# liuyuan-pal/NeRO

Measured on AMD Instinct MI355X. Metric: training rays/sec (Stage-I shape, 128 samples/ray), higher is better.
Workload: dtype f32 (dense layers: fp32 operands carried as exact / block-scaled 16-bit plane pairs or triples on the bf16/fp16 matrix pipe with fp32 accumulation, fp32-grade error; modes {'fwd': 'f16x3', 'tan': 'f16x3', 'bwd': 'f16x3', 'dw': 'f16x3'}); 1 GPU; GlossySynthetic 'bell' Stage-I shape, 4096 rays x (64+64+32) samples per GPU, training-schedule step 25000; rays_per_gpu=4096, parallelism=dp1, optimizer=adam(fused), streams=3, f16_paired_mask=3, fg_table=reference asset (tests/golden/fg_lut_ref.npz)

## Files before the change

### nero_amd/csrc/mlp_f16_util.h

```cpp
#pragma once

#ifdef F16_PHASE_TIMING
__device__ unsigned long long g_phase[16];
#define PH_DECL long long ph_t = clock64(), ph_acc[8] = {0, 0, 0, 0, 0, 0, 0, 0}
#define PH(k) do { __builtin_amdgcn_sched_barrier(0); const long long t_ = clock64(); ph_acc[k] += t_ - ph_t; ph_t = t_; __builtin_amdgcn_sched_barrier(0); } while (0)
#define PH_PARAM , long long& ph_t, long long (&ph_acc)[8]
#define PH_ARG , ph_t, ph_acc
#define PH_END do { if (threadIdx.x == 0) for (int k_ = 0; k_ < 8; ++k_) atomicAdd(&g_phase[k_], (unsigned long long)ph_acc[k_]); } while (0)
#else
#define PH_PARAM
#define PH_ARG
#define PH_DECL
#define PH(k)
#define PH_END
#endif

typedef _Float16 f16x8 __attribute__((ext_vector_type(8)));
typedef _Float16 f16x2 __attribute__((ext_vector_type(2)));
typedef float f32x2 __attribute__((ext_vector_type(2)));
typedef float f32x16 __attribute__((ext_vector_type(16)));

constexpr float BETA = 100.0f;
constexpr int SA = 528;
constexpr int PLANE_A = 64 * SA;
// ... 245 lines not shown
}
#define NERO_FENCE() __builtin_amdgcn_sched_barrier(0)
#ifdef GEMM_SGB
#define NERO_KSTEP_SCHED() do { \
    __builtin_amdgcn_sched_group_barrier(0x008, 1, 0); __builtin_amdgcn_sched_group_barrier(0x100, 1, 0); \
    __builtin_amdgcn_sched_group_barrier(0x008, 1, 0); __builtin_amdgcn_sched_group_barrier(0x100, 1, 0); \
    __builtin_amdgcn_sched_group_barrier(0x008, 1, 0); __builtin_amdgcn_sched_group_barrier(0x100, 1, 0); \
    __builtin_amdgcn_sched_group_barrier(0x008, 1, 0); __builtin_amdgcn_sched_group_barrier(0x100, 1, 0); \
    __builtin_amdgcn_sched_group_barrier(0x008, 1, 0); __builtin_amdgcn_sched_group_barrier(0x020, 1, 0); \
    __builtin_amdgcn_sched_group_barrier(0x008, 1, 0); __builtin_amdgcn_sched_group_barrier(0x020, 1, 0); } while (0)
#define NERO_MID_FENCE()
#else
#define NERO_KSTEP_SCHED()
#define NERO_MID_FENCE() NERO_FENCE()
#endif

#ifndef F16_PW_N
#define F16_PW_N 3
#endif
__device__ __forceinline__ void prefetch_w(WF& wa, WF& wb, WF& wc, const uint4* wp, int n, int from = 0) {
    const int last = n - 1;
    if (from <= 0) load_w(wa, wp, 0);
    if (from <= 1) load_w(wb, wp, 1 < last ? 1 : last);
    if (from <= 2) load_w(wc, wp, 2 < last ? 2 : last);
}
__device__ __forceinline__ void gemm_f16x3_loop(f32x16 (&aH)[2], f32x16 (&aL)[2], const uint4* wp, const char* xp, int half_bytes,
                                           int plane_bytes, int n, bool pre, WF& wa, WF& wb, WF& wc) {
    if (n <= 0) return;
    WF wd;
    XF xa, xb;
    const int last = n - 1;
#define NERO_CL(c) ((c) < last ? (c) : last)
    prefetch_w(wa, wb, wc, wp, n, pre ? F16_PW_N : 0);
    load_x(xa, xp, half_bytes, plane_bytes, 0);
    NERO_FENCE();
    for (int c = 0; c < n; c += 4) {
        load_w(wd, wp, NERO_CL(c + 3)); load_x(xb, xp, half_bytes, plane_bytes, NERO_CL(c + 1)); NERO_MID_FENCE();
        ops_compute(aH, aL, wa, xa); NERO_KSTEP_SCHED(); NERO_FENCE();
        if (c + 1 < n) {
            load_w(wa, wp, NERO_CL(c + 4)); load_x(xa, xp, half_bytes, plane_bytes, NERO_CL(c + 2)); NERO_MID_FENCE();
            ops_compute(aH, aL, wb, xb); NERO_KSTEP_SCHED(); NERO_FENCE();
        }
        if (c + 2 < n) {
            load_w(wb, wp, NERO_CL(c + 5)); load_x(xb, xp, half_bytes, plane_bytes, NERO_CL(c + 3)); NERO_MID_FENCE();
            ops_compute(aH, aL, wc, xa); NERO_KSTEP_SCHED(); NERO_FENCE();
        }
        if (c + 3 < n) {
            load_w(wc, wp, NERO_CL(c + 6)); load_x(xa, xp, half_bytes, plane_bytes, NERO_CL(c + 4)); NERO_MID_FENCE();
            ops_compute(aH, aL, wd, xb); NERO_KSTEP_SCHED(); NERO_FENCE();
        }
    }
#undef NERO_CL
}
__device__ __forceinline__ void gemm_f16x3_loop(f32x16 (&aH)[2], f32x16 (&aL)[2], const uint4* wp, const char* xp, int half_bytes,
                                           int plane_bytes, int n) {
    WF wa, wb, wc;
    gemm_f16x3_loop(aH, aL, wp, xp, half_bytes, plane_bytes, n, false, wa, wb, wc);
}


__device__ __forceinline__ void gemm_f16x3_lean(f32x16 (&aH)[2], f32x16 (&aL)[2], const uint4* wp, const char* xp, int half_bytes,
                                                int plane_bytes, int n) {
    if (n <= 0) return;
    WF w0, w1, w2;
    XF xa, xb;
    const int last = n - 1;
#define NERO_CL(c) ((c) < last ? (c) : last)
    load_w(w0, wp, 0);
    load_w(w1, wp, NERO_CL(1));
    load_x(xa, xp, half_bytes, plane_bytes, 0);
    NERO_FENCE();
    for (int c = 0; c < n; c += 6) {
        load_w(w2, wp, NERO_CL(c + 2)); load_x(xb, xp, half_bytes, plane_bytes, NERO_CL(c + 1)); NERO_FENCE();
        ops_compute(aH, aL, w0, xa); NERO_FENCE();
        if (c + 1 < n) { load_w(w0, wp, NERO_CL(c + 3)); load_x(xa, xp, half_bytes, plane_bytes, NERO_CL(c + 2)); NERO_FENCE(); ops_compute(aH, aL, w1, xb); NERO_FENCE(); }
        if (c + 2 < n) { load_w(w1, wp, NERO_CL(c + 4)); load_x(xb, xp, half_bytes, plane_bytes, NERO_CL(c + 3)); NERO_FENCE(); ops_compute(aH, aL, w2, xa); NERO_FENCE(); }
        if (c + 3 < n) { load_w(w2, wp, NERO_CL(c + 5)); load_x(xa, xp, half_bytes, plane_bytes, NERO_CL(c + 4)); NERO_FENCE(); ops_compute(aH, aL, w0, xb); NERO_FENCE(); }
        if (c + 4 < n) { load_w(w0, wp, NERO_CL(c + 6)); load_x(xb, xp, half_bytes, plane_bytes, NERO_CL(c + 5)); NERO_FENCE(); ops_compute(aH, aL, w1, xa); NERO_FENCE(); }
        if (c + 5 < n) { load_w(w1, wp, NERO_CL(c + 7)); load_x(xa, xp, half_bytes, plane_bytes, NERO_CL(c + 6)); NERO_FENCE(); ops_compute(aH, aL, w2, xb); NERO_FENCE(); }
    }
#undef NERO_CL
}

template <int V> struct IC { static constexpr int value = V; };
template <int I, int N, class F> __device__ __forceinline__ void static_for(F&& f) {
    if constexpr (I < N) { f(IC<I>{}); static_for<I + 1, N>(f); }
}
#ifndef GEMM_XD
#define GEMM_XD 1
#endif
#ifndef GEMM_WD
#define GEMM_WD 3
#endif
template <int N, class F>
__device__ __forceinline__ void gemm_f16x3_fixed_hook(f32x16 (&aH)[2], f32x16 (&aL)[2], const uint4* wp, const char* xp, int half_bytes,
                                                      int plane_bytes, F&& hook) {
    constexpr int XD = GEMM_XD, XN = XD + 1, WD = GEMM_WD, WN = WD + 1;
    WF w[WN];
    XF x[XN];
    static_for<0, WD>([&](auto c) { if (c.value < N) load_w(w[c.value], wp, c.value); });
    static_for<0, XD>([&](auto c) { if (c.value < N) load_x(x[c.value], xp, half_bytes, plane_bytes, c.value); });
    NERO_FENCE();
    static_for<0, N>([&](auto cc) {
        constexpr int c = cc.value;
        if (c + WD < N) load_w(w[(c + WD) % WN], wp, c + WD);
        if (c + XD < N) load_x(x[(c + XD) % XN], xp, half_bytes, plane_bytes, c + XD);
        hook(cc);
        NERO_MID_FENCE();
        ops_compute(aH, aL, w[c % WN], x[c % XN]);
        if (c + WD < N && c + XD < N) NERO_KSTEP_SCHED();
        NERO_FENCE();
    });
}
template <int N>
__device__ __forceinline__ void gemm_f16x3_fixed(f32x16 (&aH)[2], f32x16 (&aL)[2], const uint4* wp, const char* xp, int half_bytes,
                                                 int plane_bytes) {
    gemm_f16x3_fixed_hook<N>(aH, aL, wp, xp, half_bytes, plane_bytes, [](auto) {});
}

__device__ __forceinline__ void gemm_f16x3(f32x16 (&aH)[2], f32x16 (&aL)[2], const uint4* wp, const char* xp, int half_bytes,
                                           int plane_bytes, int n) {
#ifdef GEMM_ASSUME16
    gemm_f16x3_fixed<16>(aH, aL, wp, xp, half_bytes, plane_bytes); return;
#endif
    gemm_f16x3_loop(aH, aL, wp, xp, half_bytes, plane_bytes, n);
}

__device__ __forceinline__ void zero2(f32x16 (&acc)[2]) {
#pragma unroll
    for (int r = 0; r < 2; ++r)
#pragma unroll
        for (int v = 0; v < 16; ++v) acc[r][v] = 0.f;
}

#ifdef NERO_SHFL_LDS
__device__ __forceinline__ float max_xor32(float m) { return fmaxf(m, __shfl_xor(m, 32)); }
__device__ __forceinline__ unsigned other_half(unsigned v, int h) { (void)h; return __shfl_xor(v, 32); }
__device__ __forceinline__ float max_8lanes(float m) { m = fmaxf(m, __shfl_xor(m, 1)); m = fmaxf(m, __shfl_xor(m, 2)); return fmaxf(m, __shfl_xor(m, 4)); }
__device__ __forceinline__ float max_4lanes(float m) { m = fmaxf(m, __shfl_xor(m, 1)); return fmaxf(m, __shfl_xor(m, 2)); }
__device__ __forceinline__ float sum_8lanes(float s) { s += __shfl_xor(s, 1); s += __shfl_xor(s, 2); return s + __shfl_xor(s, 4); }
#else
__device__ __forceinline__ float max_xor32(float m) {
    const auto r = __builtin_amdgcn_permlane32_swap(__float_as_uint(m), __float_as_uint(m), false, false);
    return fmaxf(__uint_as_float(r[0]), __uint_as_float(r[1]));
}
__device__ __forceinline__ unsigned other_half(unsigned v, int h) {
    const auto r = __builtin_amdgcn_permlane32_swap(v, v, false, false);
    return h ? r[0] : r[1];
}
template <int CTRL> __device__ __forceinline__ float dpp_f32(float v) {
    return __uint_as_float(__builtin_amdgcn_update_dpp(0u, __float_as_uint(v), CTRL, 0xf, 0xf, true));
}
__device__ __forceinline__ float max_4lanes(float m) { m = fmaxf(m, dpp_f32<0xB1>(m)); return fmaxf(m, dpp_f32<0x4E>(m)); }
__device__ __forceinline__ float max_8lanes(float m) { m = max_4lanes(m); return fmaxf(m, dpp_f32<0x141>(m)); }
__device__ __forceinline__ float sum_8lanes(float s) { s += dpp_f32<0xB1>(s); s += dpp_f32<0x4E>(s); return s + dpp_f32<0x141>(s); }
#endif

__device__ __forceinline__ void publish_rowmax(float* rmax, float m0, float m1, int wave, int i, int h) {
    m0 = max_xor32(m0);
    m1 = max_xor32(m1);
    if (h == 0) { rmax[i * 8 + wave] = m0; rmax[(32 + i) * 8 + wave] = m1; }
}
__device__ __forceinline__ float row_max8(const float* rmax, int row) {
    const float4 a = *reinterpret_cast<const float4*>(rmax + row * 8);
    const float4 b = *reinterpret_cast<const float4*>(rmax + row * 8 + 4);
    return fmaxf(fmaxf(fmaxf(a.x, a.y), fmaxf(a.z, a.w)), fmaxf(fmaxf(b.x, b.y), fmaxf(b.z, b.w)));
// ... 81 lines not shown
```

### nero_amd/csrc/mlp_f16p.hip

```cpp
#include <hip/hip_runtime.h>
#include <stdint.h>
#include "../../include/nero_hip.h"
#include "common.h"
#include "mlp_split.h"

namespace {

#include "mlp_f16_util.h"

#ifndef P_PA_EARLY_A
#define P_PA_EARLY_A true
#endif
#ifndef P_PA_EARLY_B
#define P_PA_EARLY_B true
#endif

struct LdsP { char* actp; float* rs_main; float* rs_aux; float* rmax; float* wsc; char* scr; };
__device__ __forceinline__ LdsP carve_p(char* smem) {
    LdsP l;
    l.actp = smem;
    l.rs_main = reinterpret_cast<float*>(smem + 2 * PLANE_A);
    l.rs_aux = l.rs_main + 64;
    l.rmax = l.rs_aux + 64;
    l.wsc = l.rmax + 64 * 8;
    l.scr = reinterpret_cast<char*>(l.wsc + 32);
    return l;
}
#ifndef NERO_F16_PW_DEFAULT
#define NERO_F16_PW_DEFAULT 4
#endif
#ifndef P_LDS_EXTRA
#define P_LDS_EXTRA 0
#endif
inline int p_lds_bytes() { return 2 * PLANE_A + LDS_SMALL_BYTES + 4 * SCRP_BYTES + P_LDS_EXTRA; }

struct Ctx { LdsP S; int wave, lane, i, h, row0, n_rows; float* scr; };

template <int NW>
__device__ __forceinline__ void load_planes_scaled_p(char* planes, float* rs, const float* __restrict__ src, int ld, int k, int row0,
                                                     int n_rows, int tid) {
    constexpr int NV = 64 / NW;
    const int r = tid / NW, q = tid % NW;
    const int k16 = (k + 15) & ~15, q4 = k16 >> 2;
    int gr = row0 + r;
    gr = gr < n_rows ? gr : n_rows - 1;
    const float* rowp = src + (size_t)gr * ld;
    float4 v[NV];
    float m = 0.f;
#pragma unroll
    for (int j = 0; j < NV; ++j) {
        const int c4 = 4 * (q + NW * j);
        v[j] = make_float4(0.f, 0.f, 0.f, 0.f);
        if (c4 < k) v[j] = *reinterpret_cast<const float4*>(rowp + c4);
        m = fmaxf(m, amax4(v[j]));
    }
    m = NW == 8 ? max_8lanes(m) : max_4lanes(m);
    const int e = scale_exp(m);
    const float inv = pow2i(-e);
#pragma unroll
    for (int j = 0; j < NV; ++j)
        if (q + NW * j < q4) store_planes4h(planes + r * SA + (q + NW * j) * 8, PLANE_A, scale4(v[j], inv));
    if (q == 0) rs[r] = pow2i(e);
}

template <int NW>
__device__ __forceinline__ void aux_row_scales_p(float* rs, const float* __restrict__ src, int ld, int k, int row0, int n_rows, int tid) {
    const int r = tid / NW, q = tid % NW;
    int gr = row0 + r;
    gr = gr < n_rows ? gr : n_rows - 1;
    const float* rowp = src + (size_t)gr * ld;
    float m = 0.f;
    for (int c4 = 4 * q; c4 < k; c4 += 4 * NW) m = fmaxf(m, amax4(*reinterpret_cast<const float4*>(rowp + c4)));
    m = NW == 8 ? max_8lanes(m) : max_4lanes(m);
    if (q == 0) rs[r] = pow2i(scale_exp(m));
}

struct RawX { float4 a0, a1, b0, b1; };
__device__ __forceinline__ void load_raw(RawX& o, const float* p0, const float* p1, int c, int h, int k) {
    const int c0 = 16 * c + 8 * h;
    const float4 z = make_float4(0.f, 0.f, 0.f, 0.f);
    o.a0 = c0 < k ? *reinterpret_cast<const float4*>(p0 + c0) : z;
    o.a1 = c0 + 4 < k ? *reinterpret_cast<const float4*>(p0 + c0 + 4) : z;
    o.b0 = c0 < k ? *reinterpret_cast<const float4*>(p1 + c0) : z;
    o.b1 = c0 + 4 < k ? *reinterpret_cast<const float4*>(p1 + c0 + 4) : z;
}
__device__ __forceinline__ void split8(uint4& hp, uint4& lp, float4 a, float4 b, float inv) {
    split2h(a.x * inv, a.y * inv, hp.x, lp.x);
    split2h(a.z * inv, a.w * inv, hp.y, lp.y);
    split2h(b.x * inv, b.y * inv, hp.z, lp.z);
    split2h(b.z * inv, b.w * inv, hp.w, lp.w);
}
__device__ __forceinline__ void raw_to_x(XF& x, const RawX& r, float inv0, float inv1) {
    split8(x.xh0, x.xl0, r.a0, r.a1, inv0);
    split8(x.xh1, x.xl1, r.b0, r.b1, inv1);
}
__device__ __forceinline__ void gemm_aux_global(f32x16 (&aH)[2], f32x16 (&aL)[2], const uint4* wp, const float* __restrict__ aux, int ld,
                                                int k, int n, const Ctx& c, float inv0, float inv1) {
    if (n <= 0) return;
    int g0 = c.row0 + c.i, g1 = c.row0 + 32 + c.i;
    g0 = g0 < c.n_rows ? g0 : c.n_rows - 1;
    g1 = g1 < c.n_rows ? g1 : c.n_rows - 1;
    const float* p0 = aux + (size_t)g0 * ld;
    const float* p1 = aux + (size_t)g1 * ld;
    WF wa, wb;
    RawX ra, rb;
    XF x;
    load_w(wa, wp, 0);
    load_raw(ra, p0, p1, 0, c.h, k);
    for (int s = 0; s < n; s += 2) {
        if (s + 1 < n) { load_w(wb, wp, s + 1); load_raw(rb, p0, p1, s + 1, c.h, k); }
        NERO_FENCE();
        raw_to_x(x, ra, inv0, inv1);
        ops_compute(aH, aL, wa, x);
        NERO_FENCE();
        if (s + 1 < n) {
            if (s + 2 < n) { load_w(wa, wp, s + 2); load_raw(ra, p0, p1, s + 2, c.h, k); }
            NERO_FENCE();
            raw_to_x(x, rb, inv0, inv1);
            ops_compute(aH, aL, wb, x);
            NERO_FENCE();
        }
    }
}

template <int NW>
__device__ __forceinline__ void gemm_tile(f32x16 (&aH)[2], f32x16 (&aL)[2], float (&U)[2], const Ctx& c, int t, const float* w_main,
                                          const float* w_aux, float wsc_main, float wsc_aux, int sm, int sx, const float* aux, int ld_aux,
                                          int k_aux_cols) {
    if (sx > 0) {
        const float wsc = wsc_aux;
        const float ra0 = c.S.rs_aux[c.i], ra1 = c.S.rs_aux[32 + c.i];
        gemm_aux_global(aH, aL, reinterpret_cast<const uint4*>(reinterpret_cast<const char*>(w_aux) + HDR_BYTES) + (size_t)t * sx * 128 + c.lane,
                        aux, ld_aux, k_aux_cols, sx, c, 1.f / ra0, 1.f / ra1);
        U[0] = wsc * ra0;
        U[1] = wsc * ra1;
    }
    if (sm > 0) {
        const float wsc = wsc_main;
        const float u0 = wsc * c.S.rs_main[c.i], u1 = wsc * c.S.rs_main[32 + c.i];
        if (sx > 0) {
            const float r0 = U[0] / u0, r1 = U[1] / u1;
#pragma unroll
            for (int v = 0; v < 16; ++v) {
                aH[0][v] *= r0; aH[1][v] *= r1;
#ifdef F16_TWO_ACC
                aL[0][v] *= r0; aL[1][v] *= r1;
#endif
            }
        }
        U[0] = u0;
        U[1] = u1;
        const uint4* wp = reinterpret_cast<const uint4*>(reinterpret_cast<const char*>(w_main) + HDR_BYTES) + (size_t)t * sm * 128 + c.lane;
        if (NW == 8) gemm_f16x3_lean(aH, aL, wp, c.S.actp + c.i * SA + 16 * c.h, 32 * SA, PLANE_A, sm);
        else gemm_f16x3(aH, aL, wp, c.S.actp + c.i * SA + 16 * c.h, 32 * SA, PLANE_A, sm);
    }
}

template <int NW>
__device__ __forceinline__ void eval_head_p(const char* planes, const float* rs, const float* __restrict__ w, const float* __restrict__ b,
                                            float* __restrict__ out, int n_head, int hk, int row0, int tid) {
    const int q = tid & 7;
#pragma unroll
    for (int pass = 0; pass < 8 / NW; ++pass) {
        const int r = (tid >> 3) + 32 * pass;
        float s[4] = {0.f, 0.f, 0.f, 0.f};
        for (int c4 = 4 * q; c4 < hk; c4 += 32) {
            const float4 x = load_planes4h(planes + r * SA + c4 * 2, PLANE_A);
#pragma unroll
            for (int j = 0; j < 4; ++j)
                if (j < n_head) {
                    const float4 ww = *reinterpret_cast<const float4*>(w + j * NERO_HID + c4);
                    s[j] = fmaf(x.x, ww.x, fmaf(x.y, ww.y, fmaf(x.z, ww.z, fmaf(x.w, ww.w, s[j]))));
                }
        }
#pragma unroll
        for (int j = 0; j < 4; ++j) s[j] = sum_8lanes(s[j]);
        if (q == 0) {
            const float sc = rs[r];
#pragma unroll
            for (int j = 0; j < 4; ++j)
                if (j < n_head) out[(size_t)(row0 + r) * 4 + j] = s[j] * sc + (b ? b[j] : 0.f);
        }
    }
}

template <int NW>
__device__ __forceinline__ void commit_planes_p(const Ctx& c, const float4 (&v0)[2][4], const float4 (&v1)[2][4], bool live0, bool live1) {
    __syncthreads();
    const int e0 = scale_exp(row_max8(c.S.rmax, c.i)), e1 = scale_exp(row_max8(c.S.rmax, 32 + c.i));
    const float inv0 = pow2i(-e0), inv1 = pow2i(-e1);
    if (live0) {
        char* dst = c.S.actp + c.i * SA + (32 * c.wave + 4 * c.h) * 2;
#pragma unroll
        for (int g = 0; g < 4; ++g) {
            store_planes4h(dst + 16 * g, PLANE_A, scale4(v0[0][g], inv0));
            store_planes4h(dst + 32 * SA + 16 * g, PLANE_A, scale4(v0[1][g], inv1));
        }
    }
    if (NW == 4 && live1) {
        char* dst = c.S.actp + c.i * SA + (32 * (c.wave + NW) + 4 * c.h) * 2;
#pragma unroll
        for (int g = 0; g < 4; ++g) {
            store_planes4h(dst + 16 * g, PLANE_A, scale4(v1[0][g], inv0));
            store_planes4h(dst + 32 * SA + 16 * g, PLANE_A, scale4(v1[1][g], inv1));
        }
    }
    if (c.wave == 0 && c.h == 0) { c.S.rs_main[c.i] = pow2i(e0); c.S.rs_main[32 + c.i] = pow2i(e1); }
    __syncthreads();
}

template <int NW>
__device__ __forceinline__ Ctx make_ctx(char* smem, int n_rows) {
    Ctx c;
    c.S = carve_p(smem);
    c.lane = threadIdx.x & 63;
    c.wave = __builtin_amdgcn_readfirstlane(threadIdx.x >> 6);
    c.i = c.lane & 31;
    c.h = c.lane >> 5;
    c.row0 = blockIdx.x * 64;
    c.n_rows = n_rows;
    c.scr = reinterpret_cast<float*>(c.S.scr + c.wave * (NW == 8 ? SCRP_BYTES / 2 : SCRP_BYTES));
    return c;
}

template <int ACT>
__device__ __forceinline__ void fwd_values(const f32x16 (&aH)[2], const f32x16 (&aL)[2], const float4 (&bq)[4], const float (&U)[2],
                                           float4 (&val)[2][4], float (&m)[2]) {
#pragma unroll
    for (int r = 0; r < 2; ++r) {
        m[r] = 0.f;
#pragma unroll
        for (int g = 0; g < 4; ++g) {
            float4 v;
            v.x = act_fwd<ACT>(fmaf(ACCV(aH, aL, r, 4 * g), U[r], bq[g].x));
            v.y = act_fwd<ACT>(fmaf(ACCV(aH, aL, r, 4 * g + 1), U[r], bq[g].y));
            v.z = act_fwd<ACT>(fmaf(ACCV(aH, aL, r, 4 * g + 2), U[r], bq[g].z));
            v.w = act_fwd<ACT>(fmaf(ACCV(aH, aL, r, 4 * g + 3), U[r], bq[g].w));
            val[r][g] = v;
            m[r] = fmaxf(m[r], amax4(v));
        }
    }
}

template <int NW>
__device__ __forceinline__ void fwd_tile(const nero_fwd_chain& ch, const nero_fwd_layer& L, int l, const Ctx& c, int t, float4 (&val)[2][4],
                                         float (&m)[2] PH_PARAM) {
    m[0] = m[1] = 0.f;
    if (t < L.n_tiles) {
        f32x16 aH[2], aL[2];
        zero2(aH);
        zero2(aL);
        float4 bq[4];
        auto load_bias = [&]() {
#pragma unroll
            for (int g = 0; g < 4; ++g)
                bq[g] = L.bias ? *reinterpret_cast<const float4*>(L.bias + 32 * t + 8 * g + 4 * c.h) : make_float4(0.f, 0.f, 0.f, 0.f);
        };
        if (NW == 4) load_bias();
        float U[2] = {1.f, 1.f};
        PH(1);
        gemm_tile<NW>(aH, aL, U, c, t, L.w_main, L.w_aux, c.S.wsc[2 * l], c.S.wsc[2 * l + 1], L.k_main >> 4, L.k_aux >> 4, ch.aux, ch.ld_aux, ch.k_aux);
        if (NW == 8) { NERO_FENCE(); load_bias(); }
        PH(2);
        if (L.act == NERO_ACT_RELU) fwd_values<NERO_ACT_RELU>(aH, aL, bq, U, val, m);
        else if (L.act == NERO_ACT_SOFTPLUS100) fwd_values<NERO_ACT_SOFTPLUS100>(aH, aL, bq, U, val, m);
        else fwd_values<NERO_ACT_NONE>(aH, aL, bq, U, val, m);
        PH(3);
        if (L.save) {
            float* sblock = L.save + (size_t)c.row0 * NERO_HID + 32 * t;
            acc_to_global_rows<64 / NW>(c.scr, val[0], sblock, c.lane);
            acc_to_global_rows<64 / NW>(c.scr, val[1], sblock + (size_t)32 * NERO_HID, c.lane);
        }
        if (L.relu_mask) {
#pragma unroll
            for (int r = 0; r < 2; ++r) {
                unsigned bits = 0u;
#pragma unroll
                for (int g = 0; g < 4; ++g) {
                    bits |= (val[r][g].x > 0.f ? 1u : 0u) << (4 * g);
                    bits |= (val[r][g].y > 0.f ? 1u : 0u) << (4 * g + 1);
                    bits |= (val[r][g].z > 0.f ? 1u : 0u) << (4 * g + 2);
                    bits |= (val[r][g].w > 0.f ? 1u : 0u) << (4 * g + 3);
                }
                const unsigned other = other_half(bits, c.h);
                if (c.h == 0) L.relu_mask[(size_t)(c.row0 + 32 * r + c.i) * 8 + t] = bits | (other << 16);
            }
        }
    }
    publish_rowmax(c.S.rmax, m[0], m[1], t, c.i, c.h);
    PH(4);
}

template <int NW>
__global__ __launch_bounds__(NW * 64, NW / 2) void fwd_p_kernel(nero_fwd_chain ch, int n_rows) {
    extern __shared__ __attribute__((aligned(16))) char smem[];
    const Ctx c = make_ctx<NW>(smem, n_rows);
    const int tid = threadIdx.x;
    PH_DECL;
#ifdef F16_PHASE_TIMING
    const long long ph_start = ph_t;
#endif
    WscRegs wr;
    wsc_request(wr, ch, [](const nero_fwd_layer& Lx, const float*& pm, const float*& pa) { pm = Lx.k_main > 0 && Lx.n_tiles > 0 ? Lx.w_main : nullptr; pa = Lx.k_aux > 0 && Lx.n_tiles > 0 ? Lx.w_aux : nullptr; });
    if (ch.init) load_planes_scaled_p<NW>(c.S.actp, c.S.rs_main, ch.init, ch.ld_init, ch.k_init, c.row0, n_rows, tid);
    if (ch.aux) aux_row_scales_p<NW>(c.S.rs_aux, ch.aux, ch.ld_aux, ch.k_aux, c.row0, n_rows, tid);
    wsc_commit(c.S.wsc, wr, tid);
    __syncthreads();
    PH(0);
    for (int l = 0; l < ch.n_layers; ++l) {
        const nero_fwd_layer L = load_layer(ch, l);
        if (L.n_head > 0) eval_head_p<NW>(c.S.actp, c.S.rs_main, L.head_w, L.head_b, L.head_out, L.n_head, L.head_k, c.row0, tid);
        if (L.n_tiles == 0) continue;
        float4 v0[2][4], v1[2][4];
        float m0[2], m1[2];
        fwd_tile<NW>(ch, L, l, c, c.wave, v0, m0 PH_ARG);
        if (NW == 4) fwd_tile<NW>(ch, L, l, c, c.wave + NW, v1, m1 PH_ARG);
        commit_planes_p<NW>(c, v0, v1, c.wave < L.n_tiles, c.wave + NW < L.n_tiles);
        PH(5);
    }
#ifdef F16_PHASE_TIMING
    ph_acc[7] = clock64() - ph_start;
    ph_acc[6] = 0;
#endif
    PH_END;
}

template <int NW>
__device__ __forceinline__ void tan_tile(const nero_tan_chain& ch, const nero_tan_layer& L, int l, const Ctx& c, int t, float4 (&val)[2][4],
                                         float (&m)[2]) {
    m[0] = m[1] = 0.f;
    if (t < L.n_tiles) {
        const size_t goff = (size_t)(c.row0 + c.i) * NERO_HID + 32 * t + 4 * c.h;
        const size_t boff = (size_t)c.row0 * NERO_HID + 32 * t;
        const bool want_inj = L.inj != nullptr;
        f32x16 aH[2], aL[2];
        zero2(aH);
        zero2(aL);
        float U[2] = {1.f, 1.f};
        gemm_tile<NW>(aH, aL, U, c, t, L.w_main, L.w_aux, c.S.wsc[2 * l], c.S.wsc[2 * l + 1], L.k_main >> 4, L.k_aux >> 4, ch.aux, ch.ld_aux, ch.k_aux);
        NERO_FENCE();
        float4 pa[2][4], pg[2][4];
#pragma unroll
        for (int r = 0; r < 2; ++r)
#pragma unroll
            for (int g = 0; g < 4; ++g) {
                pa[r][g] = *reinterpret_cast<const float4*>(L.a_saved + goff + (size_t)r * 32 * NERO_HID + 8 * g);
                pg[r][g] = make_float4(0.f, 0.f, 0.f, 0.f);
            }
        if (want_inj) {
#pragma unroll
            for (int r = 0; r < 2; ++r)
#pragma unroll
                for (int g = 0; g < 4; ++g) pg[r][g] = *reinterpret_cast<const float4*>(L.gbar + goff + (size_t)r * 32 * NERO_HID + 8 * g);
        }
        float* scr = c.scr;
#pragma unroll
        for (int r = 0; r < 2; ++r) {
            const bool live = (c.row0 + 32 * r + c.i) < c.n_rows;
            float4 ijq[4], adq[4];
#pragma unroll
            for (int g = 0; g < 4; ++g) {
                const float4 a = pa[r][g], gb = pg[r][g];
                float4 ad, ij;
                tan_elem(a.x, ACCV(aH, aL, r, 4 * g) * U[r], gb.x, live, ad.x, ij.x);
                tan_elem(a.y, ACCV(aH, aL, r, 4 * g + 1) * U[r], gb.y, live, ad.y, ij.y);
                tan_elem(a.z, ACCV(aH, aL, r, 4 * g + 2) * U[r], gb.z, live, ad.z, ij.z);
                tan_elem(a.w, ACCV(aH, aL, r, 4 * g + 3) * U[r], gb.w, live, ad.w, ij.w);
                val[r][g] = ad;
                m[r] = fmaxf(m[r], amax4(ad));
                adq[g] = live ? ad : make_float4(0.f, 0.f, 0.f, 0.f);
                ijq[g] = ij;
            }
            acc_to_global_rows<64 / NW>(scr, adq, L.adot + boff + (size_t)r * 32 * NERO_HID, c.lane);
            if (want_inj) acc_to_global_rows<64 / NW>(scr, ijq, L.inj + boff + (size_t)r * 32 * NERO_HID, c.lane);
        }
    }
    publish_rowmax(c.S.rmax, m[0], m[1], t, c.i, c.h);
}

template <int NW>
__global__ __launch_bounds__(NW * 64, NW / 2) void tan_p_kernel(nero_tan_chain ch, int n_rows) {
    extern __shared__ __attribute__((aligned(16))) char smem[];
    const Ctx c = make_ctx<NW>(smem, n_rows);
    const int tid = threadIdx.x;
    WscRegs wr;
    wsc_request(wr, ch, [](const nero_tan_layer& Lx, const float*& pm, const float*& pa) { pm = Lx.k_main > 0 ? Lx.w_main : nullptr; pa = Lx.k_aux > 0 ? Lx.w_aux : nullptr; });
    if (ch.init) load_planes_scaled_p<NW>(c.S.actp, c.S.rs_main, ch.init, ch.ld_init, ch.k_init, c.row0, n_rows, tid);
    if (ch.aux) aux_row_scales_p<NW>(c.S.rs_aux, ch.aux, ch.ld_aux, ch.k_aux, c.row0, n_rows, tid);
    wsc_commit(c.S.wsc, wr, tid);
    __syncthreads();
    for (int l = 0; l < ch.n_layers; ++l) {
        const nero_tan_layer L = load_layer(ch, l);
        float4 v0[2][4], v1[2][4];
        float m0[2], m1[2];
        tan_tile<NW>(ch, L, l, c, c.wave, v0, m0);
        if (NW == 4) tan_tile<NW>(ch, L, l, c, c.wave + NW, v1, m1);
        commit_planes_p<NW>(c, v0, v1, c.wave < L.n_tiles, c.wave + NW < L.n_tiles);
    }
}

__device__ __forceinline__ void combine_acc(float4 (&gq)[2][4], const f32x16 (&aH)[2], const f32x16 (&aL)[2], const float (&u)[2]) {
#pragma unroll
    for (int r = 0; r < 2; ++r)
#pragma unroll
        for (int g = 0; g < 4; ++g)
            gq[r][g] = make_float4(ACCV(aH, aL, r, 4 * g) * u[r], ACCV(aH, aL, r, 4 * g + 1) * u[r],
                                   ACCV(aH, aL, r, 4 * g + 2) * u[r], ACCV(aH, aL, r, 4 * g + 3) * u[r]);
}

template <bool PA_EARLY, int NW, bool MASKS>
__device__ __forceinline__ void bwd_tile(const nero_bwd_chain& ch, const nero_bwd_layer& L, int l, const Ctx& c, int t, bool first, float rs0, float rs1,
                                         float4 (&val)[2][4], float (&m)[2]) {
    m[0] = m[1] = 0.f;
    const bool live_t = t < L.k_main_tiles;
    const int fbase = 32 * t + 4 * c.h;
    const size_t goff = (size_t)(c.row0 + c.i) * NERO_HID + fbase;
    const size_t boff = (size_t)c.row0 * NERO_HID + 32 * t;
    const int steps = L.n_out >> 4;
    const bool has_inj = !MASKS && !first && L.inj != nullptr;
    const char* xp = c.S.actp + c.i * SA + 16 * c.h;
    float4 pa[2][4];
    auto load_pa = [&]() {
        if (first || !live_t) return;
        if (MASKS && L.act_prev != NERO_ACT_RELU) return;
        if (MASKS || (L.mask_prev && L.act_prev == NERO_ACT_RELU)) {
#pragma unroll
            for (int r = 0; r < 2; ++r) {
                const unsigned bits = L.mask_prev[(size_t)(c.row0 + 32 * r + c.i) * 8 + t] >> (16 * c.h);
#pragma unroll
                for (int g = 0; g < 4; ++g)
                    pa[r][g] = make_float4((bits >> (4 * g)) & 1u ? 1.f : 0.f, (bits >> (4 * g + 1)) & 1u ? 1.f : 0.f,
                                           (bits >> (4 * g + 2)) & 1u ? 1.f : 0.f, (bits >> (4 * g + 3)) & 1u ? 1.f : 0.f);
            }
        } else if (!MASKS) {
#pragma unroll
            for (int r = 0; r < 2; ++r)
#pragma unroll
                for (int g = 0; g < 4; ++g) pa[r][g] = *reinterpret_cast<const float4*>(L.a_prev + goff + (size_t)r * 32 * NERO_HID + 8 * g);
        }
    };
    float4 gq[2][4];
    if (L.n_out > 0) {
        f32x16 aH[2], aL[2];
        if (ch.d_aux && L.w_aux_t && t < L.k_aux_tiles) {
            zero2(aH);
            zero2(aL);
            const float wsc = c.S.wsc[2 * l + 1];
            if (NW == 8) gemm_f16x3_lean(aH, aL, reinterpret_cast<const uint4*>(reinterpret_cast<const char*>(L.w_aux_t) + HDR_BYTES) + (size_t)t * steps * 128 + c.lane, xp, 32 * SA, PLANE_A, steps);
            else gemm_f16x3(aH, aL, reinterpret_cast<const uint4*>(reinterpret_cast<const char*>(L.w_aux_t) + HDR_BYTES) + (size_t)t * steps * 128 + c.lane,
                       xp, 32 * SA, PLANE_A, steps);
            const float u[2] = {wsc * rs0, wsc * rs1};
            combine_acc(gq, aH, aL, u);
#pragma unroll
            for (int r = 0; r < 2; ++r)
#pragma unroll
                for (int g = 0; g < 4; ++g) {
                    const int f = fbase + 8 * g;
                    if (f < ch.ld_daux) *reinterpret_cast<float4*>(ch.d_aux + (size_t)(c.row0 + 32 * r + c.i) * ch.ld_daux + f) = gq[r][g];
                }
        }
        if (!live_t || (first && !ch.d_init)) { publish_rowmax(c.S.rmax, 0.f, 0.f, t, c.i, c.h); return; }
        if (PA_EARLY) {
            load_pa();
            NERO_FENCE();
        }
        zero2(aH);
        zero2(aL);
        const float wsc = c.S.wsc[2 * l];
        if (NW == 8) gemm_f16x3_lean(aH, aL, reinterpret_cast<const uint4*>(reinterpret_cast<const char*>(L.w_main_t) + HDR_BYTES) + (size_t)t * steps * 128 + c.lane, xp, 32 * SA, PLANE_A, steps);
        else gemm_f16x3(aH, aL, reinterpret_cast<const uint4*>(reinterpret_cast<const char*>(L.w_main_t) + HDR_BYTES) + (size_t)t * steps * 128 + c.lane,
                   xp, 32 * SA, PLANE_A, steps);
        const float u[2] = {wsc * rs0, wsc * rs1};
        combine_acc(gq, aH, aL, u);
        if (first) {
            if (ch.d_init) {
                const int ldi = ch.ld_dinit;
#pragma unroll
                for (int r = 0; r < 2; ++r)
#pragma unroll
                    for (int g = 0; g < 4; ++g) {
                        const int f = fbase + 8 * g;
                        if (f < ldi) {
                            float4 v = gq[r][g];
                            float4* dstp = reinterpret_cast<float4*>(ch.d_init + (size_t)(c.row0 + 32 * r + c.i) * ldi + f);
                            if (ch.accumulate_dinit) { const float4 o = *dstp; v.x += o.x; v.y += o.y; v.z += o.z; v.w += o.w; }
                            *dstp = v;
                        }
                    }
            }
            return;
        }
    } else {
        if (!live_t) { publish_rowmax(c.S.rmax, 0.f, 0.f, t, c.i, c.h); return; }
        if (PA_EARLY) load_pa();
#pragma unroll
        for (int g = 0; g < 4; ++g) {
            gq[0][g] = scale4(load_planes4h(c.S.actp + c.i * SA + (fbase + 8 * g) * 2, PLANE_A), rs0);
            gq[1][g] = scale4(load_planes4h(c.S.actp + (32 + c.i) * SA + (fbase + 8 * g) * 2, PLANE_A), rs1);
        }
    }
    if (!PA_EARLY) {
        NERO_FENCE();
        load_pa();
    }
    float4 ijp[2][4];
#pragma unroll
    for (int r = 0; r < 2; ++r)
#pragma unroll
        for (int g = 0; g < 4; ++g) ijp[r][g] = make_float4(0.f, 0.f, 0.f, 0.f);
    if (L.act_prev == NERO_ACT_RELU) bwd_values_h<NERO_ACT_RELU, false>(gq, pa, goff, has_inj, L, c.row0, c.i, fbase, c.n_rows, val, m, ijp);
    else if (!MASKS && L.act_prev == NERO_ACT_SOFTPLUS100) bwd_values_h<NERO_ACT_SOFTPLUS100, false>(gq, pa, goff, has_inj, L, c.row0, c.i, fbase, c.n_rows, val, m, ijp);
    else bwd_values_h<NERO_ACT_NONE, false>(gq, pa, goff, has_inj, L, c.row0, c.i, fbase, c.n_rows, val, m, ijp);
    if (L.delta_prev) {
        acc_to_global_rows<64 / NW>(c.scr, val[0], L.delta_prev + boff, c.lane);
        acc_to_global_rows<64 / NW>(c.scr, val[1], L.delta_prev + boff + (size_t)32 * NERO_HID, c.lane);
    }
    publish_rowmax(c.S.rmax, m[0], m[1], t, c.i, c.h);
}

template <int NW, bool MASKS>
__global__ __launch_bounds__(NW * 64, NW / 2) void bwd_p_kernel(nero_bwd_chain ch, int n_rows) {
    extern __shared__ __attribute__((aligned(16))) char smem[];
    const Ctx c = make_ctx<NW>(smem, n_rows);
    const int tid = threadIdx.x;
    WscRegs wr;
    wsc_request(wr, ch, [](const nero_bwd_layer& Lx, const float*& pm, const float*& pa) { pm = Lx.n_out > 0 ? Lx.w_main_t : nullptr; pa = Lx.n_out > 0 ? Lx.w_aux_t : nullptr; });
    if (ch.dy) load_planes_scaled_p<NW>(c.S.actp, c.S.rs_main, ch.dy, ch.ld_dy, ch.k_dy, c.row0, n_rows, tid);
    else {
        for (int idx = tid; idx < 2 * PLANE_A / 16; idx += NW * 64) reinterpret_cast<uint4*>(c.S.actp)[idx] = make_uint4(0u, 0u, 0u, 0u);
        if (tid < 64) c.S.rs_main[tid] = 1.f;
    }
    wsc_commit(c.S.wsc, wr, tid);
    __syncthreads();
    for (int l = ch.n_layers - 1; l >= 0; --l) {
        const nero_bwd_layer L = load_layer(ch, l);
        const bool first = (L.a_prev == nullptr);
        if (first && ch.d_init == nullptr && !(ch.d_aux && L.w_aux_t)) break;
        if (first && L.n_out == 0) break;
        const float rs0 = c.S.rs_main[c.i], rs1 = c.S.rs_main[32 + c.i];
        float4 v0[2][4], v1[2][4];
        float m0[2], m1[2];
        bwd_tile<P_PA_EARLY_A, NW, MASKS>(ch, L, l, c, c.wave, first, rs0, rs1, v0, m0);
        if (NW == 4) bwd_tile<P_PA_EARLY_B, NW, MASKS>(ch, L, l, c, c.wave + NW, first, rs0, rs1, v1, m1);
        if (first) break;
        commit_planes_p<NW>(c, v0, v1, c.wave < L.k_main_tiles, c.wave + NW < L.k_main_tiles);
    }
}

}

#include <stdio.h>
#include <stdlib.h>
#ifdef F16_PHASE_TIMING
extern "C" int nero_debug_phases_p(unsigned long long* out16, int reset) {
    hipDeviceSynchronize();
    if (out16) hipMemcpyFromSymbol(out16, HIP_SYMBOL(g_phase), sizeof(unsigned long long) * 16);
    if (reset) { unsigned long long z[16] = {0}; hipMemcpyToSymbol(HIP_SYMBOL(g_phase), z, sizeof(z)); }
    return 0;
}
#endif
static void report_occupancy(const void* f, const char* name) {
    if (!getenv("NERO_DEBUG_OCC")) return;
    for (int lds = 32768; lds <= 81920; lds += 2048 * 3) {
        int nb = -1;
        hipError_t e = hipOccupancyMaxActiveBlocksPerMultiprocessor(&nb, f, 256, lds);
        fprintf(stderr, "[nero] %s: dynamic LDS %d -> %d workgroups per CU (err %d)\n", name, lds, nb, (int)e);
    }
// ... 58 lines not shown
```

Measured before the change: 148,300 rays/s.

## Compute paired output tiles in one GEMM pass sharing activation loads

When a wave owns two output tiles (NW==4), the forward and tangent chains now run a dual GEMM that loads each activation fragment once and feeds it to two weight streams and two accumulator sets, instead of two separate GEMM passes. Epilogues are factored out so both tiles reuse them. The goal is to halve activation LDS/global reads and the loop overhead per tile pair. The cost is doubled accumulator and weight-fragment registers, which may lower occupancy or cause spills. A small asm trick also keeps the bwd store indices in VGPRs.

```diff
diff --git a/nero_amd/csrc/mlp_f16_util.h b/nero_amd/csrc/mlp_f16_util.h
--- a/nero_amd/csrc/mlp_f16_util.h
+++ b/nero_amd/csrc/mlp_f16_util.h
@@ -351,6 +351,39 @@
 #undef NERO_CL
 }
 
+struct WF2 { WF a, b; };
+__device__ __forceinline__ void load_w2(WF2& o, const uint4* wp0, const uint4* wp1, int c) {
+    load_w(o.a, wp0, c);
+    load_w(o.b, wp1, c);
+}
+__device__ __forceinline__ void ops_compute2(f32x16 (&aH0)[2], f32x16 (&aL0)[2], f32x16 (&aH1)[2], f32x16 (&aL1)[2], const WF2& w, const XF& x) {
+    ops_compute(aH0, aL0, w.a, x);
+    ops_compute(aH1, aL1, w.b, x);
+}
+__device__ __forceinline__ void gemm_f16x3_dual(f32x16 (&aH0)[2], f32x16 (&aL0)[2], f32x16 (&aH1)[2], f32x16 (&aL1)[2], const uint4* wp0,
+                                                const uint4* wp1, const char* xp, int half_bytes, int plane_bytes, int n) {
+    if (n <= 0) return;
+    WF2 w0, w1, w2;
+    XF xa, xb;
+    const int last = n - 1;
+#define NERO_CL(c) ((c) < last ? (c) : last)
+#define NERO_K2(W, X) NERO_MID_FENCE(); ops_compute2(aH0, aL0, aH1, aL1, W, X); NERO_FENCE()
+    load_w2(w0, wp0, wp1, 0);
+    load_w2(w1, wp0, wp1, NERO_CL(1));
+    load_x(xa, xp, half_bytes, plane_bytes, 0);
+    NERO_FENCE();
+    for (int c = 0; c < n; c += 6) {
+        load_w2(w2, wp0, wp1, NERO_CL(c + 2)); load_x(xb, xp, half_bytes, plane_bytes, NERO_CL(c + 1)); NERO_K2(w0, xa);
+        if (c + 1 < n) { load_w2(w0, wp0, wp1, NERO_CL(c + 3)); load_x(xa, xp, half_bytes, plane_bytes, NERO_CL(c + 2)); NERO_K2(w1, xb); }
+        if (c + 2 < n) { load_w2(w1, wp0, wp1, NERO_CL(c + 4)); load_x(xb, xp, half_bytes, plane_bytes, NERO_CL(c + 3)); NERO_K2(w2, xa); }
+        if (c + 3 < n) { load_w2(w2, wp0, wp1, NERO_CL(c + 5)); load_x(xa, xp, half_bytes, plane_bytes, NERO_CL(c + 4)); NERO_K2(w0, xb); }
+        if (c + 4 < n) { load_w2(w0, wp0, wp1, NERO_CL(c + 6)); load_x(xb, xp, half_bytes, plane_bytes, NERO_CL(c + 5)); NERO_K2(w1, xa); }
+        if (c + 5 < n) { load_w2(w1, wp0, wp1, NERO_CL(c + 7)); load_x(xa, xp, half_bytes, plane_bytes, NERO_CL(c + 6)); NERO_K2(w2, xb); }
+    }
+#undef NERO_K2
+#undef NERO_CL
+}
+
 template <int V> struct IC { static constexpr int value = V; };
 template <int I, int N, class F> __device__ __forceinline__ void static_for(F&& f) {
     if constexpr (I < N) { f(IC<I>{}); static_for<I + 1, N>(f); }
diff --git a/nero_amd/csrc/mlp_f16p.hip b/nero_amd/csrc/mlp_f16p.hip
--- a/nero_amd/csrc/mlp_f16p.hip
+++ b/nero_amd/csrc/mlp_f16p.hip
@@ -34,6 +34,7 @@
 #endif
 inline int p_lds_bytes() { return 2 * PLANE_A + LDS_SMALL_BYTES + 4 * SCRP_BYTES + P_LDS_EXTRA; }
 
+#define P_LOCAL_V(x) asm volatile("" : "+v"(x))
 struct Ctx { LdsP S; int wave, lane, i, h, row0, n_rows; float* scr; };
 
 template <int NW>
@@ -123,6 +124,81 @@
     }
 }
 
+__device__ __forceinline__ void gemm_aux_global2(f32x16 (&aH0)[2], f32x16 (&aL0)[2], f32x16 (&aH1)[2], f32x16 (&aL1)[2], const uint4* wp0,
+                                                 const uint4* wp1, const float* __restrict__ aux, int ld, int k, int n, const Ctx& c, float inv0,
+                                                 float inv1) {
+    if (n <= 0) return;
+    int g0 = c.row0 + c.i, g1 = c.row0 + 32 + c.i;
+    g0 = g0 < c.n_rows ? g0 : c.n_rows - 1;
+    g1 = g1 < c.n_rows ? g1 : c.n_rows - 1;
+    const float* p0 = aux + (size_t)g0 * ld;
+    const float* p1 = aux + (size_t)g1 * ld;
+    WF2 wa, wb;
+    RawX ra, rb;
+    XF x;
+    load_w2(wa, wp0, wp1, 0);
+    load_raw(ra, p0, p1, 0, c.h, k);
+    for (int s = 0; s < n; s += 2) {
+        if (s + 1 < n) { load_w2(wb, wp0, wp1, s + 1); load_raw(rb, p0, p1, s + 1, c.h, k); }
+        NERO_FENCE();
+        raw_to_x(x, ra, inv0, inv1);
+        ops_compute2(aH0, aL0, aH1, aL1, wa, x);
+        NERO_FENCE();
+        if (s + 1 < n) {
+            if (s + 2 < n) { load_w2(wa, wp0, wp1, s + 2); load_raw(ra, p0, p1, s + 2, c.h, k); }
+            NERO_FENCE();
+            raw_to_x(x, rb, inv0, inv1);
+            ops_compute2(aH0, aL0, aH1, aL1, wb, x);
+            NERO_FENCE();
+        }
+    }
+}
+
+#ifndef P_DUAL_TILE
+#ifdef F16_TWO_ACC
+#define P_DUAL_TILE 0
+#else
+#define P_DUAL_TILE 1
+#endif
+#endif
+#ifndef P_DUAL_TILE_TAN
+#define P_DUAL_TILE_TAN P_DUAL_TILE
+#endif
+
+template <int NW>
+__device__ __forceinline__ void gemm_tile2(f32x16 (&aH0)[2], f32x16 (&aL0)[2], f32x16 (&aH1)[2], f32x16 (&aL1)[2], float (&U)[2], const Ctx& c,
+                                           int t, const float* w_main, const float* w_aux, float wsc_main, float wsc_aux, int sm, int sx,
+                                           const float* aux, int ld_aux, int k_aux_cols) {
+    if (sx > 0) {
+        const float wsc = wsc_aux;
+        const float ra0 = c.S.rs_aux[c.i], ra1 = c.S.rs_aux[32 + c.i];
+        const uint4* wp = reinterpret_cast<const uint4*>(reinterpret_cast<const char*>(w_aux) + HDR_BYTES) + (size_t)t * sx * 128 + c.lane;
+        gemm_aux_global2(aH0, aL0, aH1, aL1, wp, wp + (size_t)NW * sx * 128, aux, ld_aux, k_aux_cols, sx, c, 1.f / ra0, 1.f / ra1);
+        U[0] = wsc * ra0;
+        U[1] = wsc * ra1;
+    }
+    if (sm > 0) {
+        const float wsc = wsc_main;
+        const float u0 = wsc * c.S.rs_main[c.i], u1 = wsc * c.S.rs_main[32 + c.i];
+        if (sx > 0) {
+            const float r0 = U[0] / u0, r1 = U[1] / u1;
+#pragma unroll
+            for (int v = 0; v < 16; ++v) {
+                aH0[0][v] *= r0; aH0[1][v] *= r1;
+                aH1[0][v] *= r0; aH1[1][v] *= r1;
+#ifdef F16_TWO_ACC
+                aL0[0][v] *= r0; aL0[1][v] *= r1;
+                aL1[0][v] *= r0; aL1[1][v] *= r1;
+#endif
+            }
+        }
+        U[0] = u0;
+        U[1] = u1;
+        const uint4* wp = reinterpret_cast<const uint4*>(reinterpret_cast<const char*>(w_main) + HDR_BYTES) + (size_t)t * sm * 128 + c.lane;
+        gemm_f16x3_dual(aH0, aL0, aH1, aL1, wp, wp + (size_t)NW * sm * 128, c.S.actp + c.i * SA + 16 * c.h, 32 * SA, PLANE_A, sm);
+    }
+}
+
 template <int NW>
 __device__ __forceinline__ void gemm_tile(f32x16 (&aH)[2], f32x16 (&aL)[2], float (&U)[2], const Ctx& c, int t, const float* w_main,
                                           const float* w_aux, float wsc_main, float wsc_aux, int sm, int sx, const float* aux, int ld_aux,
@@ -242,6 +318,43 @@
     }
 }
 
+__device__ __forceinline__ void fwd_load_bias(float4 (&bq)[4], const nero_fwd_layer& L, const Ctx& c, int t) {
+#pragma unroll
+    for (int g = 0; g < 4; ++g)
+        bq[g] = L.bias ? *reinterpret_cast<const float4*>(L.bias + 32 * t + 8 * g + 4 * c.h) : make_float4(0.f, 0.f, 0.f, 0.f);
+}
+
+template <int NW>
+__device__ __forceinline__ void fwd_epilogue(const nero_fwd_layer& L, const Ctx& c, int t, const f32x16 (&aH)[2], const f32x16 (&aL)[2],
+                                             const float4 (&bq)[4], const float (&U)[2], float4 (&val)[2][4], float (&m)[2] PH_PARAM) {
+    if (L.act == NERO_ACT_RELU) fwd_values<NERO_ACT_RELU>(aH, aL, bq, U, val, m);
+    else if (L.act == NERO_ACT_SOFTPLUS100) fwd_values<NERO_ACT_SOFTPLUS100>(aH, aL, bq, U, val, m);
+    else fwd_values<NERO_ACT_NONE>(aH, aL, bq, U, val, m);
+    PH(3);
+    if (L.save) {
+        float* sblock = L.save + (size_t)c.row0 * NERO_HID + 32 * t;
+        acc_to_global_rows<64 / NW>(c.scr, val[0], sblock, c.lane);
+        acc_to_global_rows<64 / NW>(c.scr, val[1], sblock + (size_t)32 * NERO_HID, c.lane);
+    }
+    if (L.relu_mask) {
+#pragma unroll
+        for (int r = 0; r < 2; ++r) {
+            unsigned bits = 0u;
+#pragma unroll
+            for (int g = 0; g < 4; ++g) {
+                bits |= (val[r][g].x > 0.f ? 1u : 0u) << (4 * g);
+                bits |= (val[r][g].y > 0.f ? 1u : 0u) << (4 * g + 1);
+                bits |= (val[r][g].z > 0.f ? 1u : 0u) << (4 * g + 2);
+                bits |= (val[r][g].w > 0.f ? 1u : 0u) << (4 * g + 3);
+            }
+            const unsigned other = other_half(bits, c.h);
+            if (c.h == 0) L.relu_mask[(size_t)(c.row0 + 32 * r + c.i) * 8 + t] = bits | (other << 16);
+        }
+    }
+    publish_rowmax(c.S.rmax, m[0], m[1], t, c.i, c.h);
+    PH(4);
+}
+
 template <int NW>
 __device__ __forceinline__ void fwd_tile(const nero_fwd_chain& ch, const nero_fwd_layer& L, int l, const Ctx& c, int t, float4 (&val)[2][4],
                                          float (&m)[2] PH_PARAM) {
@@ -251,44 +364,38 @@
         zero2(aH);
         zero2(aL);
         float4 bq[4];
-        auto load_bias = [&]() {
-#pragma unroll
-            for (int g = 0; g < 4; ++g)
-                bq[g] = L.bias ? *reinterpret_cast<const float4*>(L.bias + 32 * t + 8 * g + 4 * c.h) : make_float4(0.f, 0.f, 0.f, 0.f);
-        };
-        if (NW == 4) load_bias();
+        if (NW == 4) fwd_load_bias(bq, L, c, t);
         float U[2] = {1.f, 1.f};
         PH(1);
         gemm_tile<NW>(aH, aL, U, c, t, L.w_main, L.w_aux, c.S.wsc[2 * l], c.S.wsc[2 * l + 1], L.k_main >> 4, L.k_aux >> 4, ch.aux, ch.ld_aux, ch.k_aux);
-        if (NW == 8) { NERO_FENCE(); load_bias(); }
+        if (NW == 8) { NERO_FENCE(); fwd_load_bias(bq, L, c, t); }
         PH(2);
-        if (L.act == NERO_ACT_RELU) fwd_values<NERO_ACT_RELU>(aH, aL, bq, U, val, m);
-        else if (L.act == NERO_ACT_SOFTPLUS100) fwd_values<NERO_ACT_SOFTPLUS100>(aH, aL, bq, U, val, m);
-        else fwd_values<NERO_ACT_NONE>(aH, aL, bq, U, val, m);
-        PH(3);
-        if (L.save) {
-            float* sblock = L.save + (size_t)c.row0 * NERO_HID + 32 * t;
-            acc_to_global_rows<64 / NW>(c.scr, val[0], sblock, c.lane);
-            acc_to_global_rows<64 / NW>(c.scr, val[1], sblock + (size_t)32 * NERO_HID, c.lane);
-        }
-        if (L.relu_mask) {
-#pragma unroll
-            for (int r = 0; r < 2; ++r) {
-                unsigned bits = 0u;
-#pragma unroll
-                for (int g = 0; g < 4; ++g) {
-                    bits |= (val[r][g].x > 0.f ? 1u : 0u) << (4 * g);
-                    bits |= (val[r][g].y > 0.f ? 1u : 0u) << (4 * g + 1);
-                    bits |= (val[r][g].z > 0.f ? 1u : 0u) << (4 * g + 2);
-                    bits |= (val[r][g].w > 0.f ? 1u : 0u) << (4 * g + 3);
-                }
-                const unsigned other = other_half(bits, c.h);
-                if (c.h == 0) L.relu_mask[(size_t)(c.row0 + 32 * r + c.i) * 8 + t] = bits | (other << 16);
-            }
-        }
-    }
-    publish_rowmax(c.S.rmax, m[0], m[1], t, c.i, c.h);
-    PH(4);
+        fwd_epilogue<NW>(L, c, t, aH, aL, bq, U, val, m PH_ARG);
+    } else {
+        publish_rowmax(c.S.rmax, 0.f, 0.f, t, c.i, c.h);
+        PH(4);
+    }
+}
+
+template <int NW>
+__device__ __forceinline__ void fwd_tile_pair(const nero_fwd_chain& ch, const nero_fwd_layer& L, int l, const Ctx& c, int t, float4 (&v0)[2][4],
+                                              float4 (&v1)[2][4], float (&m0)[2], float (&m1)[2] PH_PARAM) {
+    f32x16 aH0[2], aL0[2], aH1[2], aL1[2];
+    zero2(aH0);
+    zero2(aL0);
+    zero2(aH1);
+    zero2(aL1);
+    float4 bq[4];
+    fwd_load_bias(bq, L, c, t);
+    float U[2] = {1.f, 1.f};
+    PH(1);
+    gemm_tile2<NW>(aH0, aL0, aH1, aL1, U, c, t, L.w_main, L.w_aux, c.S.wsc[2 * l], c.S.wsc[2 * l + 1], L.k_main >> 4, L.k_aux >> 4, ch.aux,
+                   ch.ld_aux, ch.k_aux);
+    float4 bq1[4];
+    fwd_load_bias(bq1, L, c, t + NW);
+    PH(2);
+    fwd_epilogue<NW>(L, c, t, aH0, aL0, bq, U, v0, m0 PH_ARG);
+    fwd_epilogue<NW>(L, c, t + NW, aH1, aL1, bq1, U, v1, m1 PH_ARG);
 }
 
 template <int NW>
@@ -313,8 +420,16 @@
         if (L.n_tiles == 0) continue;
         float4 v0[2][4], v1[2][4];
         float m0[2], m1[2];
+#if P_DUAL_TILE
+        if (NW == 4 && c.wave + NW < L.n_tiles) fwd_tile_pair<NW>(ch, L, l, c, c.wave, v0, v1, m0, m1 PH_ARG);
+        else {
+            fwd_tile<NW>(ch, L, l, c, c.wave, v0, m0 PH_ARG);
+            if (NW == 4) fwd_tile<NW>(ch, L, l, c, c.wave + NW, v1, m1 PH_ARG);
+        }
+#else
         fwd_tile<NW>(ch, L, l, c, c.wave, v0, m0 PH_ARG);
         if (NW == 4) fwd_tile<NW>(ch, L, l, c, c.wave + NW, v1, m1 PH_ARG);
+#endif
         commit_planes_p<NW>(c, v0, v1, c.wave < L.n_tiles, c.wave + NW < L.n_tiles);
         PH(5);
     }
@@ -326,56 +441,80 @@
 }
 
 template <int NW>
+__device__ __forceinline__ void tan_epilogue(const nero_tan_layer& L, const Ctx& c, int t, const f32x16 (&aH)[2], const f32x16 (&aL)[2],
+                                             const float (&U)[2], float4 (&val)[2][4], float (&m)[2]) {
+    const size_t goff = (size_t)(c.row0 + c.i) * NERO_HID + 32 * t + 4 * c.h;
+    const size_t boff = (size_t)c.row0 * NERO_HID + 32 * t;
+    const bool want_inj = L.inj != nullptr;
+    m[0] = m[1] = 0.f;
+    NERO_FENCE();
+    float4 pa[2][4], pg[2][4];
+#pragma unroll
+    for (int r = 0; r < 2; ++r)
+#pragma unroll
+        for (int g = 0; g < 4; ++g) {
+            pa[r][g] = *reinterpret_cast<const float4*>(L.a_saved + goff + (size_t)r * 32 * NERO_HID + 8 * g);
+            pg[r][g] = make_float4(0.f, 0.f, 0.f, 0.f);
+        }
+    if (want_inj) {
+#pragma unroll
+        for (int r = 0; r < 2; ++r)
+#pragma unroll
+            for (int g = 0; g < 4; ++g) pg[r][g] = *reinterpret_cast<const float4*>(L.gbar + goff + (size_t)r * 32 * NERO_HID + 8 * g);
+    }
+    float* scr = c.scr;
+#pragma unroll
+    for (int r = 0; r < 2; ++r) {
+        const bool live = (c.row0 + 32 * r + c.i) < c.n_rows;
+        float4 ijq[4], adq[4];
+#pragma unroll
+        for (int g = 0; g < 4; ++g) {
+            const float4 a = pa[r][g], gb = pg[r][g];
+            float4 ad, ij;
+            tan_elem(a.x, ACCV(aH, aL, r, 4 * g) * U[r], gb.x, live, ad.x, ij.x);
+            tan_elem(a.y, ACCV(aH, aL, r, 4 * g + 1) * U[r], gb.y, live, ad.y, ij.y);
+            tan_elem(a.z, ACCV(aH, aL, r, 4 * g + 2) * U[r], gb.z, live, ad.z, ij.z);
+            tan_elem(a.w, ACCV(aH, aL, r, 4 * g + 3) * U[r], gb.w, live, ad.w, ij.w);
+            val[r][g] = ad;
+            m[r] = fmaxf(m[r], amax4(ad));
+            adq[g] = live ? ad : make_float4(0.f, 0.f, 0.f, 0.f);
+            ijq[g] = ij;
+        }
+        acc_to_global_rows<64 / NW>(scr, adq, L.adot + boff + (size_t)r * 32 * NERO_HID, c.lane);
+        if (want_inj) acc_to_global_rows<64 / NW>(scr, ijq, L.inj + boff + (size_t)r * 32 * NERO_HID, c.lane);
+    }
+    publish_rowmax(c.S.rmax, m[0], m[1], t, c.i, c.h);
+}
+
+template <int NW>
 __device__ __forceinline__ void tan_tile(const nero_tan_chain& ch, const nero_tan_layer& L, int l, const Ctx& c, int t, float4 (&val)[2][4],
                                          float (&m)[2]) {
-    m[0] = m[1] = 0.f;
     if (t < L.n_tiles) {
-        const size_t goff = (size_t)(c.row0 + c.i) * NERO_HID + 32 * t + 4 * c.h;
-        const size_t boff = (size_t)c.row0 * NERO_HID + 32 * t;
-        const bool want_inj = L.inj != nullptr;
         f32x16 aH[2], aL[2];
         zero2(aH);
         zero2(aL);
         float U[2] = {1.f, 1.f};
         gemm_tile<NW>(aH, aL, U, c, t, L.w_main, L.w_aux, c.S.wsc[2 * l], c.S.wsc[2 * l + 1], L.k_main >> 4, L.k_aux >> 4, ch.aux, ch.ld_aux, ch.k_aux);
-        NERO_FENCE();
-        float4 pa[2][4], pg[2][4];
-#pragma unroll
-        for (int r = 0; r < 2; ++r)
-#pragma unroll
-            for (int g = 0; g < 4; ++g) {
-                pa[r][g] = *reinterpret_cast<const float4*>(L.a_saved + goff + (size_t)r * 32 * NERO_HID + 8 * g);
-                pg[r][g] = make_float4(0.f, 0.f, 0.f, 0.f);
-            }
-        if (want_inj) {
-#pragma unroll
-            for (int r = 0; r < 2; ++r)
-#pragma unroll
-                for (int g = 0; g < 4; ++g) pg[r][g] = *reinterpret_cast<const float4*>(L.gbar + goff + (size_t)r * 32 * NERO_HID + 8 * g);
-        }
-        float* scr = c.scr;
-#pragma unroll
-        for (int r = 0; r < 2; ++r) {
-            const bool live = (c.row0 + 32 * r + c.i) < c.n_rows;
-            float4 ijq[4], adq[4];
-#pragma unroll
-            for (int g = 0; g < 4; ++g) {
-                const float4 a = pa[r][g], gb = pg[r][g];
-                float4 ad, ij;
-                tan_elem(a.x, ACCV(aH, aL, r, 4 * g) * U[r], gb.x, live, ad.x, ij.x);
-                tan_elem(a.y, ACCV(aH, aL, r, 4 * g + 1) * U[r], gb.y, live, ad.y, ij.y);
-                tan_elem(a.z, ACCV(aH, aL, r, 4 * g + 2) * U[r], gb.z, live, ad.z, ij.z);
-                tan_elem(a.w, ACCV(aH, aL, r, 4 * g + 3) * U[r], gb.w, live, ad.w, ij.w);
-                val[r][g] = ad;
-                m[r] = fmaxf(m[r], amax4(ad));
-                adq[g] = live ? ad : make_float4(0.f, 0.f, 0.f, 0.f);
-                ijq[g] = ij;
-            }
-            acc_to_global_rows<64 / NW>(scr, adq, L.adot + boff + (size_t)r * 32 * NERO_HID, c.lane);
-            if (want_inj) acc_to_global_rows<64 / NW>(scr, ijq, L.inj + boff + (size_t)r * 32 * NERO_HID, c.lane);
-        }
-    }
-    publish_rowmax(c.S.rmax, m[0], m[1], t, c.i, c.h);
+        tan_epilogue<NW>(L, c, t, aH, aL, U, val, m);
+    } else {
+        m[0] = m[1] = 0.f;
+        publish_rowmax(c.S.rmax, 0.f, 0.f, t, c.i, c.h);
+    }
+}
+
+template <int NW>
+__device__ __forceinline__ void tan_tile_pair(const nero_tan_chain& ch, const nero_tan_layer& L, int l, const Ctx& c, int t, float4 (&v0)[2][4],
+                                              float4 (&v1)[2][4], float (&m0)[2], float (&m1)[2]) {
+    f32x16 aH0[2], aL0[2], aH1[2], aL1[2];
+    zero2(aH0);
+    zero2(aL0);
+    zero2(aH1);
+    zero2(aL1);
+    float U[2] = {1.f, 1.f};
+    gemm_tile2<NW>(aH0, aL0, aH1, aL1, U, c, t, L.w_main, L.w_aux, c.S.wsc[2 * l], c.S.wsc[2 * l + 1], L.k_main >> 4, L.k_aux >> 4, ch.aux,
+                   ch.ld_aux, ch.k_aux);
+    tan_epilogue<NW>(L, c, t, aH0, aL0, U, v0, m0);
+    tan_epilogue<NW>(L, c, t + NW, aH1, aL1, U, v1, m1);
 }
 
 template <int NW>
@@ -393,8 +532,16 @@
         const nero_tan_layer L = load_layer(ch, l);
         float4 v0[2][4], v1[2][4];
         float m0[2], m1[2];
+#if P_DUAL_TILE_TAN
+        if (NW == 4 && c.wave + NW < L.n_tiles) tan_tile_pair<NW>(ch, L, l, c, c.wave, v0, v1, m0, m1);
+        else {
+            tan_tile<NW>(ch, L, l, c, c.wave, v0, m0);
+            if (NW == 4) tan_tile<NW>(ch, L, l, c, c.wave + NW, v1, m1);
+        }
+#else
         tan_tile<NW>(ch, L, l, c, c.wave, v0, m0);
         if (NW == 4) tan_tile<NW>(ch, L, l, c, c.wave + NW, v1, m1);
+#endif
         commit_planes_p<NW>(c, v0, v1, c.wave < L.n_tiles, c.wave + NW < L.n_tiles);
     }
 }
@@ -451,12 +598,15 @@
                        xp, 32 * SA, PLANE_A, steps);
             const float u[2] = {wsc * rs0, wsc * rs1};
             combine_acc(gq, aH, aL, u);
+            int li = c.i, lf = fbase;
+            P_LOCAL_V(li);
+            P_LOCAL_V(lf);
 #pragma unroll
             for (int r = 0; r < 2; ++r)
 #pragma unroll
                 for (int g = 0; g < 4; ++g) {
-                    const int f = fbase + 8 * g;
-                    if (f < ch.ld_daux) *reinterpret_cast<float4*>(ch.d_aux + (size_t)(c.row0 + 32 * r + c.i) * ch.ld_daux + f) = gq[r][g];
+                    const int f = lf + 8 * g;
+                    if (f < ch.ld_daux) *reinterpret_cast<float4*>(ch.d_aux + (size_t)(c.row0 + 32 * r + li) * ch.ld_daux + f) = gq[r][g];
                 }
         }
         if (!live_t || (first && !ch.d_init)) { publish_rowmax(c.S.rmax, 0.f, 0.f, t, c.i, c.h); return; }
@@ -475,14 +625,17 @@
         if (first) {
             if (ch.d_init) {
                 const int ldi = ch.ld_dinit;
+                int li = c.i, lf = fbase;
+                P_LOCAL_V(li);
+                P_LOCAL_V(lf);
 #pragma unroll
                 for (int r = 0; r < 2; ++r)
 #pragma unroll
                     for (int g = 0; g < 4; ++g) {
-                        const int f = fbase + 8 * g;
+                        const int f = lf + 8 * g;
                         if (f < ldi) {
                             float4 v = gq[r][g];
-                            float4* dstp = reinterpret_cast<float4*>(ch.d_init + (size_t)(c.row0 + 32 * r + c.i) * ldi + f);
+                            float4* dstp = reinterpret_cast<float4*>(ch.d_init + (size_t)(c.row0 + 32 * r + li) * ldi + f);
                             if (ch.accumulate_dinit) { const float4 o = *dstp; v.x += o.x; v.y += o.y; v.z += o.z; v.w += o.w; }
                             *dstp = v;
                         }
```

New measurement: 151,100 rays/s, median of 6. +1.9%, better.
